# voletiv/mcvd-pytorch

Hardware: AMD Instinct MI355X
Metric: sampled frames/sec (whole node), SMMNIST 64x64 DDPM 100-step (higher is better)
Workload: dtype f32-equivalent: f32 storage and accumulation; 58 of 58 3x3 convs, 41 of 41 1x1 convs and the attention products (head dims 32..128) as SIX bf16 piece products of operands split EXACTLY into three bf16 pieces (all 24 bits, fp32 exponent range, less than one fp32 rounding per product; tests/test_gpu_p

## Files before the change

mcvd_pytorch_amd/csrc/kernels/conv_wino3.cpp:

```cpp
#include <stdlib.h>

#include "../common.h"
#include "conv_wino3_stage.h"

namespace mcvd {

#define W3_SLOT_OFF(word) (word)

template <int COT, int PRO, bool G8, int EXP = 0>
__global__ __launch_bounds__(512) __attribute__((amdgpu_num_vgpr(86))) void conv_wino3_kernel(ConvArgs a) {
    constexpr int NT = W3_NT, CK = W3_CK, T = W3_T, BCO = 32 * COT, PP = W3_PP, VW = W3_VW, PW = W3_PW;
    constexpr int PSZ = CK * 10 * PP;
    constexpr int PBUF = PSZ + 8;
    constexpr int NPL = G8 ? 1 : 3;
    constexpr int NPV = G8 ? 4 : 9;
    constexpr int NQ = 3 * COT;
    constexpr int NA = 2 * NQ;
    constexpr int VM_A = NQ + NPL;
    constexpr int PQ = 5;
    static_assert(NA <= 18 && NA > PQ, "named-register map of conv_wino3_stage.h: v172-v180 patch, v184-v255 eighteen weight quads");
    extern __shared__ __attribute__((aligned(16))) float smem[];
    unsigned* sV = reinterpret_cast<unsigned*>(smem);
    float* sP = smem + 2 * VW;
    float* sCo = sP + 2 * PBUF;

    {
        float top;
        asm volatile("" : "={v255}"(top));
    }
    asm volatile("" :: "s"(a.x0), "s"(a.x1), "s"(a.coef), "s"(a.wpb), "s"(a.B), "s"(a.H), "s"(a.W), "s"(a.Cin), "s"(a.CinP), "s"(a.C0),
                 "s"(a.C1), "s"(a.CoutP), "s"(a.ksplit), "s"(a.dbg), "s"(a.wdma));
    const unsigned long long t_start = a.dbg ? __builtin_amdgcn_s_memtime() : 0ull;
    const int tid = threadIdx.x, lane = tid & 63, wave = tid >> 6, l31 = lane & 31, half = lane >> 5;
    const int H = a.H, W = a.W, HW = H * W, Cin = a.Cin;
    const int nch_all = a.CinP / CK;
    const int ksp = a.ksplit >= 2 ? a.ksplit : 1, kh = ksp >= 2 ? (int)blockIdx.y : 0;
    const int c_begin = kh * (nch_all / ksp), c_end = c_begin + nch_all / ksp;
    const int PC = (nch_all / ksp) * CK;
    unsigned* sOff = reinterpret_cast<unsigned*>(sCo + (G8 ? 4 : 2) * PC);
    const int rx_n = G8 ? 1 : W >> 4, ry_n = G8 ? 1 : H >> 3;
    const int nreg = G8 ? (a.B + 1) >> 1 : a.B * rx_n * ry_n;
    const int nct = a.CoutP / BCO;
    const int xcd = blockIdx.x & 7, slot = blockIdx.x >> 3;
    const int reg_id = (slot / nct) * 8 + xcd;
    const int cotile = slot - (slot / nct) * nct;
    if (reg_id >= nreg) return;
    const int b = G8 ? 2 * reg_id : reg_id / (rx_n * ry_n);
    const int rr = G8 ? 0 : reg_id - b * (rx_n * ry_n);
    const int oy0 = (rr / rx_n) * 8, ox0 = (rr % rx_n) * 16;
    const int co0 = cotile * BCO;
    const int rg = __builtin_amdgcn_readfirstlane(wave >> 2);

    constexpr int NE = G8 ? 2 : 4;
    const bool wide = !G8 && PC > 2 * NT;
    const float* co_src[4];
#pragma unroll
    for (int k = 0; k < NE; ++k) {
        co_src[k] = a.coef + ((long)b * Cin + min(CK * c_begin + tid + k * NT, Cin - 1)) * 2;
        if (G8) co_src[2 + k] = a.coef + ((long)min(b + 1, a.B - 1) * Cin + min(CK * c_begin + tid + k * NT, Cin - 1)) * 2;
    }
    if (PRO) {
        asm volatile("global_load_dwordx2 v[172:173], %0, off\n\tglobal_load_dwordx2 v[174:175], %1, off"
                     :: "v"(co_src[0]), "v"(co_src[1]) : "memory");
        if (G8 || wide)
            asm volatile("global_load_dwordx2 v[176:177], %0, off\n\tglobal_load_dwordx2 v[178:179], %1, off"
                         :: "v"(co_src[2]), "v"(co_src[3]) : "memory");
    }

    const int s_tile = tid & 31, s_cp = (tid & 255) >> 5;
    const int s_ty = G8 ? (s_tile >> 2) & 3 : s_tile >> 3, s_tx = G8 ? (s_tile & 3) + 5 * (s_tile >> 4) : s_tile & 7;
    const int p_rd = ((s_cp * 10 + 2 * s_ty + rg) * PP + 2 * s_tx) * 2;
    const int v_wr = ((8 * rg * 2 + (s_cp & 1)) * 4 + (s_cp >> 1)) * T + s_tile;

    unsigned p_pk[NPL];
#pragma unroll
    for (int sl = 0; sl < NPL; ++sl) {
        p_pk[sl] = (unsigned)PSZ | ((unsigned)CK << 12);
        unsigned off = 0;
        if (G8) {
            const int e = tid, ci = e >> 5, img = (e >> 4) & 1, r = (e >> 1) & 7, c = (e & 1) * 4;
            const bool valid = b + img < a.B;
            const int cp = (ci >> 2) * 2 + (ci & 1), ce = (ci >> 1) & 1;
            p_pk[sl] = (unsigned)(((cp * 10 + r + 1) * PP + img * 10 + c + 1) * 2 + ce) | ((unsigned)(ci + (valid ? 0 : CK)) << 12) |
                       ((unsigned)(valid ? img : 0) << 20);
            off = (unsigned)(ci * HW + r * 8 + c) * 4u;
        } else if (sl < 2) {
            const int e = sl * NT + tid;
            if (e < CK * 40) {
                const int ci = e / 40, rem = e - ci * 40, r = rem >> 2, c = (rem & 3) * 4;
                const int y = oy0 - 1 + r;
                const bool inside = y >= 0 && y < H;
                const int cp = (ci >> 2) * 2 + (ci & 1), ce = (ci >> 1) & 1;
                p_pk[sl] = (unsigned)(((cp * 10 + r) * PP + c + 1) * 2 + ce) | ((unsigned)(ci + (inside ? 0 : CK)) << 12);
                off = (unsigned)(ci * HW + min(max(y, 0), H - 1) * W + ox0 + c) * 4u;
            }
        } else if (tid < CK * 20) {
            const int e = tid, ci = e / 20, rem = e - ci * 20, r = rem >> 1, c = (rem & 1) * 17;
            const int y = oy0 - 1 + r, x = ox0 - 1 + c;
            const bool inside = y >= 0 && y < H && x >= 0 && x < W;
            const int cp = (ci >> 2) * 2 + (ci & 1), ce = (ci >> 1) & 1;
            p_pk[sl] = (unsigned)(((cp * 10 + r) * PP + c) * 2 + ce) | ((unsigned)(ci + (inside ? 0 : CK)) << 12);
            off = (unsigned)(ci * HW + min(max(y, 0), H - 1) * W + min(max(x, 0), W - 1)) * 4u;
        }
        sOff[sl * NT + tid] = off;
    }

    const int wave_u = __builtin_amdgcn_readfirstlane(wave);
    const unsigned* wr_base = reinterpret_cast<const unsigned*>(a.wpb) + ((long)cotile * (a.CinP / CK) * 16 + 2 * wave_u) * (NQ * 256);
    const unsigned wr_voff = (unsigned)lane * 16u;

#define W3_WCHUNK(ch) (wr_base + (long)(ch) * (16 * NQ * 256))
#define W3_READ_OFF(OFS) { _Pragma("unroll") for (int sl = 0; sl < NPL; ++sl) OFS[sl] = sOff[sl * NT + tid]; }
#define W3_READ_C(ch, cfv)                                                                                      \
    {                                                                                                           \
        _Pragma("unroll") for (int sl = 0; sl < NPL; ++sl) {                                                    \
            cfv[sl] = f32x2{1.0f, 0.0f};                                                                        \
            if (PRO >= 1) {                                                                                     \
                 \
                const int cch = min(((ch) - c_begin) * CK + (int)((p_pk[sl] >> 12) & (CK - 1)), PC - 1) + (G8 ? (int)((p_pk[sl] >> 20) & 1u) * PC : 0); \
                cfv[sl] = *reinterpret_cast<const f32x2*>(sCo + cch * 2);                                       \
            }                                                                                                   \
        }                                                                                                       \
    }
                                                                                         \
#define W3_VALU_PHASE(ch, RG)                                                                                   \
    {                                                                                                           \
        {                                                                                                       \
            f32x2 cfv[NPL];                                                                                     \
            unsigned ofs[NPL];                                                                                  \
            W3_TS(7)                                                                                            \
            if (!(EXP & 2)) W3_READ_C((ch) + 2, cfv)                                                            \
            if (!(EXP & 4)) W3_READ_OFF(ofs)                                                                    \
            if (!(EXP & 4)) W3_WAIT(NA)                                                                         \
            W3_TS(0)                                                                                            \
            float pv[NPV];                                                                                      \
// ... 22 lines not shown
    const bool rec = a.dbg != nullptr && wave == (a.wdma & 7);
    const bool sub = (a.wdma & 64) != 0;
    unsigned long long sp[5] = {0, 0, 0, 0, 0};
    unsigned long long tk0 = 0, tprev = 0, dt[2] = {0, 0}, rt0 = 0;
    if (rec) {
        rt0 = __builtin_amdgcn_s_memrealtime();
        tk0 = tprev = t_start;
    }
#define W3_STAMP(i)                                                                                             \
    if (rec) {                                                                                                  \
        const unsigned long long now = __builtin_amdgcn_s_memtime();                                            \
        dt[i] += now - tprev;                                                                                   \
        tprev = now;                                                                                            \
    }
#ifdef MCVD_DIAG
    const bool tsub = rec && (a.wdma & 128) != 0;
    unsigned long long ts[8] = {0, 0, 0, 0, 0, 0, 0, 0}, tsp = 0;
#define W3_TS(i)                                                                                                \
    if (tsub) {                                                                                                 \
        const unsigned long long now = __builtin_amdgcn_s_memtime();                                            \
        ts[i] += now - tsp;                                                                                     \
        tsp = now;                                                                                              \
    }
#else
#define W3_TS(i)
#endif

    int vtok = 0;
    {
        const float nodep = 0.0f;
        unsigned ofs[NPL];
        W3_READ_OFF(ofs)
        if (rec) sp[3] = __builtin_amdgcn_s_memtime() - tk0;
        W3_LOAD_PR(b, c_begin, nodep, ofs, "v[184:187]", "v[188:191]", "v192")
        W3_LOAD_PR(b, c_begin + 1, nodep, ofs, "v[194:197]", "v[198:201]", "v202")
        if (G8)
            for (int i = tid; i < 2 * PBUF; i += NT) sP[i] = 0.0f;
        if (rec) sp[0] = __builtin_amdgcn_s_memtime() - tk0;
        W3_WAIT(0)
        if (rec) sp[1] = __builtin_amdgcn_s_memtime() - tk0;
        float cdep = 0.0f;
        if (PRO) {
            f32x2 cpre[4] = {{1.0f, 0.0f}, {1.0f, 0.0f}, {1.0f, 0.0f}, {1.0f, 0.0f}};
            asm volatile("v_mov_b32 %0, v172\n\tv_mov_b32 %1, v173\n\tv_mov_b32 %2, v174\n\tv_mov_b32 %3, v175"
                         : "=v"(cpre[0].x), "=v"(cpre[0].y), "=v"(cpre[1].x), "=v"(cpre[1].y) : "s"(vtok));
            if (G8 || wide)
                asm volatile("v_mov_b32 %0, v176\n\tv_mov_b32 %1, v177\n\tv_mov_b32 %2, v178\n\tv_mov_b32 %3, v179"
                             : "=v"(cpre[2].x), "=v"(cpre[2].y), "=v"(cpre[3].x), "=v"(cpre[3].y) : "s"(vtok));
#pragma unroll
            for (int k = 0; k < NE; ++k)
                if (tid + k * NT < PC) {
                    *reinterpret_cast<f32x2*>(sCo + (tid + k * NT) * 2) = cpre[k];
                    if constexpr (G8) *reinterpret_cast<f32x2*>(sCo + (PC + tid + k * NT) * 2) = cpre[2 + k];
                }
            cdep = cpre[0].x + cpre[1].x + cpre[2].x + cpre[3].x;
        }
        W3_LOAD_P(b, c_begin + 2, cdep, ofs)
        if (PRO || G8) __syncthreads();
        if (rec) sp[4] = __builtin_amdgcn_s_memtime() - tk0;
        {
            constexpr int QR = (NA - PQ + 2 * NPV - 1) / (2 * NPV);
#define W3_HOOK0(e, v) W3_LOAD_A_RANGE(W3_WCHUNK(c_begin), PQ + (e) * QR, (PQ + ((e) + 1) * QR < NA ? PQ + ((e) + 1) * QR : NA), v)
#define W3_HOOK1(e, v) W3_LOAD_A_RANGE(W3_WCHUNK(c_begin), (PQ + (NPV + (e)) * QR < NA ? PQ + (NPV + (e)) * QR : NA), (PQ + (NPV + (e) + 1) * QR < NA ? PQ + (NPV + (e) + 1) * QR : NA), v)
            float pv0[NPV], pv1[NPV];
            f32x2 cf0[NPL], cf1[NPL];
            W3_READ_C(c_begin, cf0)
            W3_READ_C(c_begin + 1, cf1)
            W3_WRITE_PR(c_begin & 1, Cin - c_begin * CK, 0u, pv0, cf0, "v184", "v185", "v186", "v187", "v188", "v189", "v190", "v191", "v192", W3_HOOK0)
            W3_WRITE_PR((c_begin + 1) & 1, Cin - (c_begin + 1) * CK, 0u, pv1, cf1, "v194", "v195", "v196", "v197", "v198", "v199", "v200", "v201", "v202", W3_HOOK1)
#undef W3_HOOK0
#undef W3_HOOK1
            const float dep = pv0[0] + pv1[0];
            W3_LOAD_A_RANGE(W3_WCHUNK(c_begin), 0, PQ, dep)
        }
    }
    __syncthreads();
    if (rec) sp[2] = __builtin_amdgcn_s_memtime() - tk0;
    {
        f32x2 rw[3][4];
        W3_READ_R(c_begin & 1, rw)
        W3_WRITE_V(c_begin & 1, rg, rw)
    }
    __syncthreads();
    W3_STAMP(0)

    W3_WAIT(0)
    const int ph = rg;
    if (ph == 0) {
        for (int c = c_begin; c + 1 < c_end; ++c) {
            W3_VALU_PHASE(c, rg)
            W3_MFMA_PHASE(c & 1, true, W3_WCHUNK(c + 1))
            asm volatile("s_waitcnt lgkmcnt(0)\n\ts_barrier" ::: "memory");
            W3_TS(6)
        }
    } else {
        for (int c = c_begin; c + 1 < c_end; ++c) {
            W3_MFMA_PHASE(c & 1, true, W3_WCHUNK(c + 1))
            W3_VALU_PHASE(c, rg)
            asm volatile("s_waitcnt lgkmcnt(0)\n\ts_barrier" ::: "memory");
            W3_TS(6)
        }
    }
    W3_WAIT(0)
    {
// ... 196 lines not shown
```

mcvd_pytorch_amd/csrc/kernels/conv_wino3_stage.h:

```cpp
#ifdef W3_STAGE_UNDEF
#undef W3_QUADS
#undef W3_LD1
#undef W3_LD1D
#undef W3_MF1
#undef W3_LOAD_A
#undef W3_LOAD_A_PIECE
#undef W3_LOAD_A_RANGE
#undef W3_WAIT
#undef W3_LOAD_PR
#undef W3_LOAD_P
#undef W3_NOHOOK
#undef W3_WRITE_PR
#undef W3_WRITE_P
#undef W3_READ_R
#undef W3_WRITE_V
#undef W3_LOAD_B
#undef W3_PRODUCT
#undef W3_MFMA_PHASE
#undef W3_STAGE_UNDEF
#else

#include "wino_common.h"

namespace mcvd {

constexpr int W3_CK = 16;
constexpr int W3_T = 32;
constexpr int W3_NT = 512;
#ifndef MCVD_W3_PP
#define MCVD_W3_PP 24
#endif
constexpr int W3_PP = MCVD_W3_PP;
constexpr int W3_PW = 16 * 2 * 4 * W3_T;
constexpr int W3_VW = 3 * W3_PW;

}

#define W3_QUADS(X, q, A1, A2) X(0, "v[184:187]", q, A1, A2) X(1, "v[188:191]", q, A1, A2) X(2, "v[192:195]", q, A1, A2) X(3, "v[196:199]", q, A1, A2) X(4, "v[200:203]", q, A1, A2) X(5, "v[204:207]", q, A1, A2) X(6, "v[208:211]", q, A1, A2) X(7, "v[212:215]", q, A1, A2) X(8, "v[216:219]", q, A1, A2) X(9, "v[220:223]", q, A1, A2) X(10, "v[224:227]", q, A1, A2) X(11, "v[228:231]", q, A1, A2) X(12, "v[232:235]", q, A1, A2) X(13, "v[236:239]", q, A1, A2) X(14, "v[240:243]", q, A1, A2) X(15, "v[244:247]", q, A1, A2) X(16, "v[248:251]", q, A1, A2) X(17, "v[252:255]", q, A1, A2)
#define W3_LD1(K, R, q, P, UNUSED) if ((q) == K) asm volatile("global_load_dwordx4 " R ", %0, %1" :: "v"(wr_voff), "s"(P) : "memory");
#define W3_MF1(K, R, q, ACC, BV) if ((q) == K) asm volatile("v_mfma_f32_32x32x16_bf16 %0, " R ", %1, %0" : "+v"(ACC) : "v"(BV));
#define W3_LOAD_A(WPTR, i)                                                                                      \
    {                                                                                                           \
        const unsigned* ua = (WPTR) + (i) * (NQ * 256);                                                         \
        _Pragma("unroll") for (int qq = 0; qq < NQ; ++qq) { W3_QUADS(W3_LD1, (i) * NQ + qq, ua + qq * 256, 0) } \
    }
#define W3_LOAD_A_PIECE(WPTR, i, pc)                                                                            \
    {                                                                                                           \
        const unsigned* ua = (WPTR) + (i) * (NQ * 256);                                                         \
        _Pragma("unroll") for (int ct = 0; ct < COT; ++ct) { W3_QUADS(W3_LD1, (i) * NQ + ct * 3 + (pc), ua + (ct * 3 + (pc)) * 256, 0) } \
    }
#define W3_LD1D(K, R, q, P, DEP) if ((q) == K) asm volatile("global_load_dwordx4 " R ", %0, %1" :: "v"(wr_voff), "s"(P), "v"(DEP) : "memory");
#define W3_LOAD_A_RANGE(WPTR, Q0, Q1, DEP)                                                                      \
    {                                                                                                           \
        const unsigned* ua = (WPTR);                                                                            \
        _Pragma("unroll") for (int qq = (Q0); qq < (Q1); ++qq) { W3_QUADS(W3_LD1D, qq, ua + qq * 256, DEP) }    \
    }
#define W3_WAIT(N) asm volatile("s_waitcnt vmcnt(%1)\n\ts_mov_b32 %0, 0" : "=s"(vtok) : "n"(N) : "memory");
#define W3_LOAD_PR(bb, ch, DEP, OFS, RA, RB, RH)                                                                \
    {                                                                                                           \
        const int cb = min((ch) * CK, Cin - 1);                                                                 \
        const unsigned lim4 = (unsigned)((Cin - cb) * HW - 4) * 4u, lim1 = (unsigned)((Cin - cb) * HW - 1) * 4u; \
        const bool second = cb >= a.C0;                                                                         \
        const float* srcb = second ? a.x1 + ((long)(bb) * a.C1 + (cb - a.C0)) * HW : a.x0 + ((long)(bb) * a.C0 + cb) * HW; \
         \
        if constexpr (G8) {                                                                                     \
            const unsigned istride = (unsigned)((second ? a.C1 : a.C0) * HW) * 4u;       \
            const unsigned o0 = min(W3_SLOT_OFF(OFS[0]), lim4) + ((p_pk[0] >> 20) & 1u) * istride;              \
            asm volatile("global_load_dwordx4 " RA ", %0, %1" :: "v"(o0), "s"(srcb), "v"(DEP) : "memory");     \
        } else {                                                                                                \
            const unsigned o0 = min(W3_SLOT_OFF(OFS[0]), lim4), o1 = min(W3_SLOT_OFF(OFS[NPL > 1 ? 1 : 0]), lim4),  \
                           o2 = min(W3_SLOT_OFF(OFS[NPL > 2 ? 2 : 0]), lim1);                                   \
            asm volatile("global_load_dwordx4 " RA ", %0, %3\n\tglobal_load_dwordx4 " RB ", %1, %3\n\tglobal_load_dword " RH ", %2, %3" \
                         :: "v"(o0), "v"(o1), "v"(o2), "s"(srcb), "v"(DEP) : "memory");                           \
        }                                                                                                       \
    }
#define W3_LOAD_P(bb, ch, DEP, OFS) W3_LOAD_PR(bb, ch, DEP, OFS, "v[172:175]", "v[176:179]", "v180")
#define W3_NOHOOK(e, v)
#define W3_WRITE_P(par, NV, FL, PV, cfv) W3_WRITE_PR(par, NV, FL, PV, cfv, "v172", "v173", "v174", "v175", "v176", "v177", "v178", "v179", "v180", W3_NOHOOK)
#define W3_WRITE_PR(par, NV, FL, PV, cfv, A0, A1, A2, A3, B0, B1, B2, B3, H0, HOOK)                             \
    {                                                                                                           \
        float* sPw = sP + ((par) ? PBUF : 0);                                                                   \
        const int nvalid = (NV);                                                                                \
         \
        if constexpr (G8) {                                                                                     \
            asm("v_fma_f32 %0, " A0 ", %4, %5\n\tv_fma_f32 %1, " A1 ", %4, %5\n\tv_fma_f32 %2, " A2 ", %4, %5\n\tv_fma_f32 %3, " A3 ", %4, %5" \
                : "=&v"(PV[0]), "=&v"(PV[1]), "=&v"(PV[2]), "=&v"(PV[3]) : "v"(cfv[0].x), "v"(cfv[0].y), "s"(vtok)); \
        } else {                                                                                                \
            asm("v_fma_f32 %0, " A0 ", %9, %10\n\tv_fma_f32 %1, " A1 ", %9, %10\n\tv_fma_f32 %2, " A2 ", %9, %10\n\tv_fma_f32 %3, " A3 ", %9, %10\n\t" \
                "v_fma_f32 %4, " B0 ", %11, %12\n\tv_fma_f32 %5, " B1 ", %11, %12\n\tv_fma_f32 %6, " B2 ", %11, %12\n\tv_fma_f32 %7, " B3 ", %11, %12\n\t" \
                "v_fma_f32 %8, " H0 ", %13, %14"                                                                  \
                : "=&v"(PV[0]), "=&v"(PV[1]), "=&v"(PV[2]), "=&v"(PV[3]), "=&v"(PV[4]), "=&v"(PV[5]), "=&v"(PV[6]), "=&v"(PV[7]), "=&v"(PV[NPV > 8 ? 8 : 0]) \
                : "v"(cfv[0].x), "v"(cfv[0].y), "v"(cfv[NPL > 1 ? 1 : 0].x), "v"(cfv[NPL > 1 ? 1 : 0].y), "v"(cfv[NPL > 2 ? 2 : 0].x), \
                  "v"(cfv[NPL > 2 ? 2 : 0].y), "s"(vtok));                                                        \
        }                                                                                                       \
        _Pragma("unroll") for (int e = 0; e < NPV; ++e) {                                                       \
            const int sl = e >> 2;                               \
            float v = PV[e];                                                                                    \
            if (PRO >= 2) v = wino_silu(v);                                                                     \
            const bool keep = (((FL) >> sl) & 1u) == 0u && (int)((p_pk[sl] >> 12) & 0xff) < min(nvalid, CK);    \
            sPw[(p_pk[sl] & 0xfff) + 2 * (e & 3)] = keep ? v : 0.0f;                                            \
            HOOK(e, v)                                                                                          \
        }                                                                                                       \
    }
#define W3_READ_R(par, RW)                                                                                      \
    {                                                                                                           \
        const f32x2* sPr = reinterpret_cast<const f32x2*>(sP + ((par) ? PBUF : 0) + p_rd);                      \
        _Pragma("unroll") for (int j = 0; j < 4; ++j) { RW[0][j] = sPr[j]; RW[1][j] = sPr[PP + j]; RW[2][j] = sPr[2 * PP + j]; } \
    }
#define W3_WRITE_V(par, RG, RW)                                                                                 \
    {                                                                                                           \
        unsigned* vdst = sV + ((par) ? VW : 0) + v_wr;                                                          \
        f32x2 mx[4], my[4];                                                                                     \
        _Pragma("unroll") for (int j = 0; j < 4; ++j) {                                                         \
            const f32x2 r0 = RW[0][j], r1 = RW[1][j], r2 = RW[2][j];                                            \
            if ((RG) == 0) { mx[j] = r0 - r2; my[j] = r1 + r2; }                                                \
            else { mx[j] = r1 - r0; my[j] = r0 - r2; }                                                          \
        }                                                                                                       \
        _Pragma("unroll") for (int row = 0; row < 2; ++row) {                                                   \
            const f32x2 m0 = row ? my[0] : mx[0], m1 = row ? my[1] : mx[1], m2 = row ? my[2] : mx[2], m3 = row ? my[3] : mx[3]; \
            const f32x2 v0 = m0 - m2, v1 = m1 + m2, v2 = m2 - m1, v3 = m1 - m3;                                 \
            _Pragma("unroll") for (int q = 0; q < 4; ++q) {                                                     \
                unsigned w1, w2, w3;                                                                            \
                wino_split3(q == 0 ? v0 : q == 1 ? v1 : q == 2 ? v2 : v3, w1, w2, w3);                          \
                vdst[(row * 4 + q) * 256] = w1;                                                                 \
                vdst[(row * 4 + q) * 256 + PW] = w2;                                                            \
                vdst[(row * 4 + q) * 256 + 2 * PW] = w3;                                                        \
            }                                                                                                   \
        }                                                                                                       \
    }
#define W3_LOAD_B(i, BQ)                                                                                        \
    {                                                                                                           \
        const unsigned* q = sVc + (((2 * wave + (i)) * 2 + half) * 4) * T + l31;                                \
        _Pragma("unroll") for (int jp = 0; jp < 4; ++jp) {                                                      \
// ... 32 lines not shown
```

mcvd_pytorch_amd/csrc/kernels/conv_wino3p.cpp:

```cpp
#include <stdlib.h>

#include "../common.h"
#include "conv_wino3_stage.h"

namespace mcvd {

constexpr int WP_NPL = 3;
constexpr int WP_MINCH = 4;

#define W3_SLOT_OFF(word) ((word) & ~3u)
#define W3_TS(i)

template <int COT, int PRO>
__global__ __launch_bounds__(512) __attribute__((amdgpu_num_vgpr(86))) void conv_wino3p_kernel(ConvArgs a) {
    constexpr int NT = W3_NT, CK = W3_CK, T = W3_T, BCO = 32 * COT, PP = W3_PP, VW = W3_VW, PW = W3_PW;
    constexpr int PSZ = CK * 10 * PP;
    constexpr int PBUF = 4096;
    static_assert(PBUF >= PSZ + 8 && PBUF >= 4 * 32 * W3_T, "patch buffer: patch + dump space, and 4 positions x 32 couts x 32 tiles of the epilogue");
    constexpr int NPL = WP_NPL, NPV = 9;
    constexpr bool G8 = false;
    constexpr int EXP = 0;
    constexpr int NQ = 3 * COT;
    constexpr int NA = 2 * NQ;
    constexpr int VM_A = NQ + NPL;
    constexpr int PQ = 5;
    constexpr long WSTR = 16L * NQ * 256;
    static_assert(NA <= 18 && NA > PQ, "named-register map of conv_wino3_stage.h: v172-v180 patch, v184-v255 eighteen weight quads");
    extern __shared__ __attribute__((aligned(16))) float smem[];
    unsigned* sV = reinterpret_cast<unsigned*>(smem);
    float* sP = smem + 2 * VW;
    float* sCo = sP + 2 * PBUF;
    unsigned* sOff = reinterpret_cast<unsigned*>(sCo + 2 * a.Cin);
    {
        float top;
        asm volatile("" : "={v255}"(top));
    }
    asm volatile("" :: "s"(a.x0), "s"(a.x1), "s"(a.coef), "s"(a.wpb), "s"(a.B), "s"(a.H), "s"(a.W), "s"(a.Cin), "s"(a.CinP), "s"(a.C0),
                 "s"(a.C1), "s"(a.CoutP), "s"(a.ksplit), "s"(a.dbg), "s"(a.wdma));
    const unsigned long long t_start = a.dbg ? __builtin_amdgcn_s_memtime() : 0ull;
    const int tid = threadIdx.x, lane = tid & 63, wave = tid >> 6, l31 = lane & 31, half = lane >> 5;
    const int H = a.H, W = a.W, HW = H * W, Cin = a.Cin;
    const int rx_n = W >> 4, rpi = rx_n * (H >> 3);
    const int nct = a.CoutP / BCO;
    const int ksp = a.ksplit >= 2 ? a.ksplit : 1;
    const int nch = (a.CinP / CK) / ksp;
    const int ips = rpi * nct * ksp;
    const int n_items = a.B * ips;
    const int it0 = (int)((long)blockIdx.x * n_items / gridDim.x), it1 = (int)((long)(blockIdx.x + 1) * n_items / gridDim.x);
    if (it0 >= it1) return;
    const int rg = __builtin_amdgcn_readfirstlane(wave >> 2);
    const int wave_u = __builtin_amdgcn_readfirstlane(wave);
#ifdef MCVD_DIAG
    if ((a.wdma >> 8) != 0 && (blockIdx.x & 1)) {
        const unsigned long long until = __builtin_amdgcn_s_memtime() + ((unsigned long long)(a.wdma >> 8) << 8);
        while (__builtin_amdgcn_s_memtime() < until) __builtin_amdgcn_s_sleep(8);
    }
#endif

    const int s_tile = tid & 31, s_cp = (tid & 255) >> 5;
    const int s_ty = s_tile >> 3, s_tx = s_tile & 7;
    const int p_rd = ((s_cp * 10 + 2 * s_ty + rg) * PP + 2 * s_tx) * 2;
    const int v_wr = ((8 * rg * 2 + (s_cp & 1)) * 4 + (s_cp >> 1)) * T + s_tile;

    unsigned p_pk[NPL];
#pragma unroll
    for (int sl = 0; sl < NPL; ++sl) {
        p_pk[sl] = (unsigned)PSZ | ((unsigned)CK << 12);
        if (sl < 2) {
            const int e = sl * NT + tid;
            if (e < CK * 40) {
                const int ci = e / 40, rem = e - ci * 40, r = rem >> 2, c = (rem & 3) * 4;
                const int cp = (ci >> 2) * 2 + (ci & 1), ce = (ci >> 1) & 1;
                p_pk[sl] = (unsigned)(((cp * 10 + r) * PP + c + 1) * 2 + ce) | ((unsigned)ci << 12);
            }
        } else if (tid < CK * 20) {
            const int e = tid, ci = e / 20, rem = e - ci * 20, r = rem >> 1, c = (rem & 1) * 17;
            const int cp = (ci >> 2) * 2 + (ci & 1), ce = (ci >> 1) & 1;
            p_pk[sl] = (unsigned)(((cp * 10 + r) * PP + c) * 2 + ce) | ((unsigned)ci << 12);
        }
    }
#define WP_SLOT_TABLE(tab, oy0, ox0, OUT)                                                                       \
    {                                                                                                           \
        int tid_s;        \
        asm volatile("v_mov_b32 %0, %1" : "=v"(tid_s) : "v"(tid));                                              \
        _Pragma("unroll") for (int sl = 0; sl < NPL; ++sl) {                                                    \
            unsigned off = 1u;                                                                                  \
            if (sl < 2) {                                                                                       \
                const int e = sl * NT + tid_s;                                                                  \
                if (e < CK * 40) {                                                                              \
                    const int ci = e / 40, rem = e - ci * 40, r = rem >> 2, c = (rem & 3) * 4;                  \
                    const int y = (oy0) - 1 + r;                                                                \
                    const bool inside = y >= 0 && y < H;                                                        \
                    off = (unsigned)(ci * HW + min(max(y, 0), H - 1) * W + (ox0) + c) * 4u + (inside ? 0u : 1u); \
                }                                                                                               \
            } else if (tid_s < CK * 20) {                                                                       \
                const int e = tid_s, ci = e / 20, rem = e - ci * 20, r = rem >> 1, c = (rem & 1) * 17;          \
                const int y = (oy0) - 1 + r, x = (ox0) - 1 + c;                                                 \
                const bool inside = y >= 0 && y < H && x >= 0 && x < W;                                         \
                off = (unsigned)(ci * HW + min(max(y, 0), H - 1) * W + min(max(x, 0), W - 1)) * 4u + (inside ? 0u : 1u); \
            }                                                                                                   \
            sOff[((tab) * NPL + sl) * NT + tid] = off;                                                          \
            OUT[sl] = off;                                                                                      \
        }                                                                                                       \
    }

    const unsigned wr_voff = (unsigned)lane * 16u;

#define WP_READ_C(ch, cfv)                                                                                      \
    {                                                                                                           \
        _Pragma("unroll") for (int sl = 0; sl < NPL; ++sl) {                                                    \
            cfv[sl] = f32x2{1.0f, 0.0f};                                                                        \
            if (PRO >= 1) {                                                                                     \
                const int cch = min((ch) * CK + (int)((p_pk[sl] >> 12) & (CK - 1)), Cin - 1);                   \
                cfv[sl] = *reinterpret_cast<const f32x2*>(sCo + cch * 2);                                       \
            }                                                                                                   \
        }                                                                                                       \
    }
#define WP_VALU_PHASE(par, CH2, CH3, TAB3, RG)                                                                  \
    {                                                                                                           \
        {                                                                                                       \
            f32x2 cfv[NPL];                                                                                     \
            unsigned ofs[NPL];                                                                                  \
            WP_READ_C(CH2, cfv)                                                                                 \
            _Pragma("unroll") for (int sl = 0; sl < NPL; ++sl) ofs[sl] = sOff[((TAB3) * NPL + sl) * NT + tid];  \
            W3_WAIT(NA)                                                                                         \
            float pv[NPV];                                                                                      \
            _Pragma("unroll") for (int e = 0; e < NPV; ++e) pv[e] = 0.0f;                                       \
            W3_WRITE_P(par, min(Cin - (CH2) * CK, CK), pfl, pv, cfv)                                            \
            pfl = (ofs[0] & 1u) | ((ofs[1] & 1u) << 1) | ((ofs[2] & 1u) << 2);                                  \
            W3_LOAD_P(b, CH3, pv[0], ofs)                                                                       \
        }                                                                                                       \
        {                                                                                                       \
            f32x2 rw[3][4];                                                                                     \
// ... 14 lines not shown
    unsigned long long tprev = t_start, dt[3] = {0, 0, 0}, rt0 = 0;
    if (rec) rt0 = __builtin_amdgcn_s_memrealtime();
#define WP_STAMP(i)                                                                                             \
    if (rec) {                                                                                                  \
        const unsigned long long now = __builtin_amdgcn_s_memtime();                                            \
        dt[i] += now - tprev;                                                                                   \
        tprev = now;                                                                                            \
    }

    const unsigned* const wpb_u = reinterpret_cast<const unsigned*>(a.wpb);
    const bool fin = ksp == 1;
    int vtok = 0;
    unsigned pfl = 0;
    int chunks_done = 0;

    int it = it0;
    while (it < it1) {
        const int b = it / ips;
        const int run_end = min(it1, (b + 1) * ips);
        {
            const int q0 = it - b * ips, kh = q0 % ksp, q1 = q0 / ksp, cotile = q1 % nct, rr = q1 / nct;
            const int oy0 = (rr / rx_n) * 8, ox0 = (rr % rx_n) * 16, cbeg = kh * nch;
            const unsigned* w0 = wpb_u + (((long)cotile * (nch * ksp) + cbeg) * 16 + 2 * wave_u) * (NQ * 256);
            const float* co_src[2];
#pragma unroll
            for (int k = 0; k < 2; ++k) co_src[k] = a.coef + ((long)b * Cin + min(tid + k * NT, Cin - 1)) * 2;
            if (PRO)
                asm volatile("global_load_dwordx2 v[172:173], %0, off\n\tglobal_load_dwordx2 v[174:175], %1, off"
                             :: "v"(co_src[0]), "v"(co_src[1]) : "memory");
            const float nodep = 0.0f;
            unsigned ofs[NPL];
            WP_SLOT_TABLE(it & 1, oy0, ox0, ofs)
            const unsigned fl0 = (ofs[0] & 1u) | ((ofs[1] & 1u) << 1) | ((ofs[2] & 1u) << 2);
            W3_LOAD_PR(b, cbeg, nodep, ofs, "v[184:187]", "v[188:191]", "v192")
            W3_LOAD_PR(b, cbeg + 1, nodep, ofs, "v[194:197]", "v[198:201]", "v202")
            W3_WAIT(0)
            float cdep = 0.0f;
            if (PRO) {
                f32x2 cpre[2];
                asm volatile("v_mov_b32 %0, v172\n\tv_mov_b32 %1, v173\n\tv_mov_b32 %2, v174\n\tv_mov_b32 %3, v175"
                             : "=v"(cpre[0].x), "=v"(cpre[0].y), "=v"(cpre[1].x), "=v"(cpre[1].y) : "s"(vtok));
#pragma unroll
                for (int k = 0; k < 2; ++k)
                    if (tid + k * NT < Cin) *reinterpret_cast<f32x2*>(sCo + (tid + k * NT) * 2) = cpre[k];
                cdep = cpre[0].x + cpre[1].x;
            }
            W3_LOAD_P(b, cbeg + 2, cdep, ofs)
            pfl = fl0;
            if (PRO) asm volatile("s_waitcnt lgkmcnt(0)\n\ts_barrier" ::: "memory");
            {
                constexpr int QR = (NA - PQ + 2 * NPV - 1) / (2 * NPV);
#define WP_HOOK0(e, v) W3_LOAD_A_RANGE(w0, PQ + (e) * QR, (PQ + ((e) + 1) * QR < NA ? PQ + ((e) + 1) * QR : NA), v)
#define WP_HOOK1(e, v) W3_LOAD_A_RANGE(w0, (PQ + (NPV + (e)) * QR < NA ? PQ + (NPV + (e)) * QR : NA), (PQ + (NPV + (e) + 1) * QR < NA ? PQ + (NPV + (e) + 1) * QR : NA), v)
                float pv0[NPV], pv1[NPV];
                f32x2 cf0[NPL], cf1[NPL];
                WP_READ_C(cbeg, cf0)
                WP_READ_C(cbeg + 1, cf1)
                W3_WRITE_PR(0, min(Cin - cbeg * CK, CK), fl0, pv0, cf0, "v184", "v185", "v186", "v187", "v188", "v189", "v190", "v191", "v192", WP_HOOK0)
                W3_WRITE_PR(1, min(Cin - (cbeg + 1) * CK, CK), fl0, pv1, cf1, "v194", "v195", "v196", "v197", "v198", "v199", "v200", "v201", "v202", WP_HOOK1)
#undef WP_HOOK0
#undef WP_HOOK1
                const float dep = pv0[0] + pv1[0];
                W3_LOAD_A_RANGE(w0, 0, PQ, dep)
            }
            asm volatile("s_waitcnt lgkmcnt(0)\n\ts_barrier" ::: "memory");
            {
                f32x2 rw[3][4];
                W3_READ_R(0, rw)
                W3_WRITE_V(0, rg, rw)
            }
            asm volatile("s_waitcnt lgkmcnt(0)\n\ts_barrier" ::: "memory");
            W3_WAIT(0)
        }
        WP_STAMP(0)
        int par = 0;
        for (; it < run_end; ++it) {
            const int q0 = it - b * ips, kh = q0 % ksp, q1 = q0 / ksp, cotile = q1 % nct, rr = q1 / nct;
            const int nx = it + 1 < run_end ? it + 1 : it;
            const int n0 = nx - b * ips, nkh = n0 % ksp, n1 = n0 / ksp, ncotile = n1 % nct, nrr = n1 / nct;
            const int cbeg = kh * nch, ncbeg = nkh * nch;
            const unsigned* wb_cur = wpb_u + (((long)cotile * (nch * ksp) + cbeg) * 16 + 2 * wave_u) * (NQ * 256);
            const unsigned* wb_nx = wpb_u + (((long)ncotile * (nch * ksp) + ncbeg) * 16 + 2 * wave_u) * (NQ * 256);
            const int tab_cur = it & 1, tab_nx = nx & 1;
            {
                unsigned dummy[NPL];
                WP_SLOT_TABLE(tab_nx, (nrr / rx_n) * 8, (nrr % rx_n) * 16, dummy)
                (void)dummy;
            }
#define WP_CHUNK_SCALARS                                                                                        \
            const int l2 = c + 2, l3 = c + 3;                                                                   \
            const int ch2 = l2 < nch ? cbeg + l2 : ncbeg + l2 - nch;                                            \
            const int ch3 = l3 < nch ? cbeg + l3 : ncbeg + l3 - nch;                                            \
            const int tab3 = l3 < nch ? tab_cur : tab_nx;                                                       \
            const unsigned* wnx = c + 1 < nch ? wb_cur + (long)(c + 1) * WSTR : wb_nx;
// ... 159 lines not shown
```

Measured before the change: 262.9.

## Remap Winograd patch slots to one quad plus two singles per thread

Result: no change. 264.8, median of 6 (+0.7%).

```diff
diff --git a/mcvd_pytorch_amd/csrc/kernels/conv_wino3.cpp b/mcvd_pytorch_amd/csrc/kernels/conv_wino3.cpp
--- a/mcvd_pytorch_amd/csrc/kernels/conv_wino3.cpp
+++ b/mcvd_pytorch_amd/csrc/kernels/conv_wino3.cpp
@@ -12,13 +12,13 @@
     constexpr int NT = W3_NT, CK = W3_CK, T = W3_T, BCO = 32 * COT, PP = W3_PP, VW = W3_VW, PW = W3_PW;
     constexpr int PSZ = CK * 10 * PP;
     constexpr int PBUF = PSZ + 8;
-    constexpr int NPL = G8 ? 1 : 3;
-    constexpr int NPV = G8 ? 4 : 9;
+    constexpr int NPL = G8 ? 1 : wino_slots::NSLOT;
+    constexpr int NPV = G8 ? 4 : wino_slots::NVAL;
     constexpr int NQ = 3 * COT;
     constexpr int NA = 2 * NQ;
     constexpr int VM_A = NQ + NPL;
-    constexpr int PQ = 5;
-    static_assert(NA <= 18 && NA > PQ, "named-register map of conv_wino3_stage.h: v172-v180 patch, v184-v255 eighteen weight quads");
+    constexpr int PQ = G8 ? 5 : 3;
+    static_assert(NA <= 18 && NA > PQ, "named-register map of conv_wino3_stage.h: v172-v176, v180 patch, v184-v255 eighteen weight quads");
     extern __shared__ __attribute__((aligned(16))) float smem[];
     unsigned* sV = reinterpret_cast<unsigned*>(smem);
     float* sP = smem + 2 * VW;
@@ -84,23 +84,11 @@
             p_pk[sl] = (unsigned)(((cp * 10 + r + 1) * PP + img * 10 + c + 1) * 2 + ce) | ((unsigned)(ci + (valid ? 0 : CK)) << 12) |
                        ((unsigned)(valid ? img : 0) << 20);
             off = (unsigned)(ci * HW + r * 8 + c) * 4u;
-        } else if (sl < 2) {
-            const int e = sl * NT + tid;
-            if (e < CK * 40) {
-                const int ci = e / 40, rem = e - ci * 40, r = rem >> 2, c = (rem & 3) * 4;
-                const int y = oy0 - 1 + r;
-                const bool inside = y >= 0 && y < H;
-                const int cp = (ci >> 2) * 2 + (ci & 1), ce = (ci >> 1) & 1;
-                p_pk[sl] = (unsigned)(((cp * 10 + r) * PP + c + 1) * 2 + ce) | ((unsigned)(ci + (inside ? 0 : CK)) << 12);
-                off = (unsigned)(ci * HW + min(max(y, 0), H - 1) * W + ox0 + c) * 4u;
-            }
-        } else if (tid < CK * 20) {
-            const int e = tid, ci = e / 20, rem = e - ci * 20, r = rem >> 1, c = (rem & 1) * 17;
-            const int y = oy0 - 1 + r, x = ox0 - 1 + c;
-            const bool inside = y >= 0 && y < H && x >= 0 && x < W;
-            const int cp = (ci >> 2) * 2 + (ci & 1), ce = (ci >> 1) & 1;
-            p_pk[sl] = (unsigned)(((cp * 10 + r) * PP + c) * 2 + ce) | ((unsigned)(ci + (inside ? 0 : CK)) << 12);
-            off = (unsigned)(ci * HW + min(max(y, 0), H - 1) * W + min(max(x, 0), W - 1)) * 4u;
+        } else {
+            const wino_slots::Slot ws = wino_slots::slot(sl, tid);
+            const wino_slots::SlotSource src = wino_slots::slot_source(ws, oy0, ox0, H, W);
+            p_pk[sl] = (unsigned)wino_slots::slot_lds_index(PP, ws) | ((unsigned)(ws.ch + (src.inside ? 0 : CK)) << 12);
+            off = src.off;
         }
         sOff[sl * NT + tid] = off;
     }
@@ -189,8 +177,13 @@
         unsigned ofs[NPL];
         W3_READ_OFF(ofs)
         if (rec) sp[3] = __builtin_amdgcn_s_memtime() - tk0;
-        W3_LOAD_PR(b, c_begin, nodep, ofs, "v[184:187]", "v[188:191]", "v192")
-        W3_LOAD_PR(b, c_begin + 1, nodep, ofs, "v[194:197]", "v[198:201]", "v202")
+        if constexpr (G8) {
+            W3_LOAD_PR(b, c_begin, nodep, ofs, "v[184:187]", "", "")
+            W3_LOAD_PR(b, c_begin + 1, nodep, ofs, "v[194:197]", "", "")
+        } else {
+            W3_LOAD_PR(b, c_begin, nodep, ofs, "v[184:187]", "v188", "v189")
+            W3_LOAD_PR(b, c_begin + 1, nodep, ofs, "v[190:193]", "v194", "v195")
+        }
         if (G8)
             for (int i = tid; i < 2 * PBUF; i += NT) sP[i] = 0.0f;
         if (rec) sp[0] = __builtin_amdgcn_s_memtime() - tk0;
@@ -217,16 +210,24 @@
         if (rec) sp[4] = __builtin_amdgcn_s_memtime() - tk0;
         {
             constexpr int QR = (NA - PQ + 2 * NPV - 1) / (2 * NPV);
-#define W3_HOOK0(e, v) W3_LOAD_A_RANGE(W3_WCHUNK(c_begin), PQ + (e) * QR, (PQ + ((e) + 1) * QR < NA ? PQ + ((e) + 1) * QR : NA), v)
-#define W3_HOOK1(e, v) W3_LOAD_A_RANGE(W3_WCHUNK(c_begin), (PQ + (NPV + (e)) * QR < NA ? PQ + (NPV + (e)) * QR : NA), (PQ + (NPV + (e) + 1) * QR < NA ? PQ + (NPV + (e) + 1) * QR : NA), v)
+#define W3_HQ(g) (G8 ? (PQ + (g) * QR < NA ? PQ + (g) * QR : NA) : PQ + (g) * (NA - PQ) / (2 * NPV))
+#define W3_HOOK0(e, v) W3_LOAD_A_RANGE(W3_WCHUNK(c_begin), W3_HQ(e), W3_HQ((e) + 1), v)
+#define W3_HOOK1(e, v) W3_LOAD_A_RANGE(W3_WCHUNK(c_begin), W3_HQ(NPV + (e)), W3_HQ(NPV + (e) + 1), v)
+            static_assert(W3_HQ(0) == PQ && W3_HQ(2 * NPV) == NA, "every quad from PQ up is requested behind a value, in order");
             float pv0[NPV], pv1[NPV];
             f32x2 cf0[NPL], cf1[NPL];
             W3_READ_C(c_begin, cf0)
             W3_READ_C(c_begin + 1, cf1)
-            W3_WRITE_PR(c_begin & 1, Cin - c_begin * CK, 0u, pv0, cf0, "v184", "v185", "v186", "v187", "v188", "v189", "v190", "v191", "v192", W3_HOOK0)
-            W3_WRITE_PR((c_begin + 1) & 1, Cin - (c_begin + 1) * CK, 0u, pv1, cf1, "v194", "v195", "v196", "v197", "v198", "v199", "v200", "v201", "v202", W3_HOOK1)
+            if constexpr (G8) {
+                W3_WRITE_PR(c_begin & 1, Cin - c_begin * CK, 0u, pv0, cf0, "v184", "v185", "v186", "v187", "", "", W3_HOOK0)
+                W3_WRITE_PR((c_begin + 1) & 1, Cin - (c_begin + 1) * CK, 0u, pv1, cf1, "v194", "v195", "v196", "v197", "", "", W3_HOOK1)
+            } else {
+                W3_WRITE_PR(c_begin & 1, Cin - c_begin * CK, 0u, pv0, cf0, "v184", "v185", "v186", "v187", "v188", "v189", W3_HOOK0)
+                W3_WRITE_PR((c_begin + 1) & 1, Cin - (c_begin + 1) * CK, 0u, pv1, cf1, "v190", "v191", "v192", "v193", "v194", "v195", W3_HOOK1)
+            }
 #undef W3_HOOK0
 #undef W3_HOOK1
+#undef W3_HQ
             const float dep = pv0[0] + pv1[0];
             W3_LOAD_A_RANGE(W3_WCHUNK(c_begin), 0, PQ, dep)
         }
diff --git a/mcvd_pytorch_amd/csrc/kernels/conv_wino3_stage.h b/mcvd_pytorch_amd/csrc/kernels/conv_wino3_stage.h
--- a/mcvd_pytorch_amd/csrc/kernels/conv_wino3_stage.h
+++ b/mcvd_pytorch_amd/csrc/kernels/conv_wino3_stage.h
@@ -21,6 +21,7 @@
 #else
 
 #include "wino_common.h"
+#include "wino_slots.h"
 
 namespace mcvd {
 
@@ -33,6 +34,7 @@
 constexpr int W3_PP = MCVD_W3_PP;
 constexpr int W3_PW = 16 * 2 * 4 * W3_T;
 constexpr int W3_VW = 3 * W3_PW;
+static_assert(W3_CK == wino_slots::CK && W3_NT == wino_slots::NT && wino_slots::lds_exact(W3_PP), "the slot map's chunk, thread count and patch pitch are the kernels'");
 
 }
 
@@ -68,16 +70,16 @@
             const unsigned o0 = min(W3_SLOT_OFF(OFS[0]), lim4) + ((p_pk[0] >> 20) & 1u) * istride;              \
             asm volatile("global_load_dwordx4 " RA ", %0, %1" :: "v"(o0), "s"(srcb), "v"(DEP) : "memory");     \
         } else {                                                                                                \
-            const unsigned o0 = min(W3_SLOT_OFF(OFS[0]), lim4), o1 = min(W3_SLOT_OFF(OFS[NPL > 1 ? 1 : 0]), lim4),  \
+            const unsigned o0 = min(W3_SLOT_OFF(OFS[0]), lim4), o1 = min(W3_SLOT_OFF(OFS[NPL > 1 ? 1 : 0]), lim1),  \
                            o2 = min(W3_SLOT_OFF(OFS[NPL > 2 ? 2 : 0]), lim1);                                   \
-            asm volatile("global_load_dwordx4 " RA ", %0, %3\n\tglobal_load_dwordx4 " RB ", %1, %3\n\tglobal_load_dword " RH ", %2, %3" \
+            asm volatile("global_load_dwordx4 " RA ", %0, %3\n\tglobal_load_dword " RB ", %1, %3\n\tglobal_load_dword " RH ", %2, %3" \
                          :: "v"(o0), "v"(o1), "v"(o2), "s"(srcb), "v"(DEP) : "memory");                           \
         }                                                                                                       \
     }
-#define W3_LOAD_P(bb, ch, DEP, OFS) W3_LOAD_PR(bb, ch, DEP, OFS, "v[172:175]", "v[176:179]", "v180")
+#define W3_LOAD_P(bb, ch, DEP, OFS) W3_LOAD_PR(bb, ch, DEP, OFS, "v[172:175]", "v176", "v180")
 #define W3_NOHOOK(e, v)
-#define W3_WRITE_P(par, NV, FL, PV, cfv) W3_WRITE_PR(par, NV, FL, PV, cfv, "v172", "v173", "v174", "v175", "v176", "v177", "v178", "v179", "v180", W3_NOHOOK)
-#define W3_WRITE_PR(par, NV, FL, PV, cfv, A0, A1, A2, A3, B0, B1, B2, B3, H0, HOOK)                             \
+#define W3_WRITE_P(par, NV, FL, PV, cfv) W3_WRITE_PR(par, NV, FL, PV, cfv, "v172", "v173", "v174", "v175", "v176", "v180", W3_NOHOOK)
+#define W3_WRITE_PR(par, NV, FL, PV, cfv, A0, A1, A2, A3, S1, S2, HOOK)                                         \
     {                                                                                                           \
         float* sPw = sP + ((par) ? PBUF : 0);                                                                   \
         const int nvalid = (NV);                                                                                \
@@ -86,19 +88,18 @@
             asm("v_fma_f32 %0, " A0 ", %4, %5\n\tv_fma_f32 %1, " A1 ", %4, %5\n\tv_fma_f32 %2, " A2 ", %4, %5\n\tv_fma_f32 %3, " A3 ", %4, %5" \
                 : "=&v"(PV[0]), "=&v"(PV[1]), "=&v"(PV[2]), "=&v"(PV[3]) : "v"(cfv[0].x), "v"(cfv[0].y), "s"(vtok)); \
         } else {                                                                                                \
-            asm("v_fma_f32 %0, " A0 ", %9, %10\n\tv_fma_f32 %1, " A1 ", %9, %10\n\tv_fma_f32 %2, " A2 ", %9, %10\n\tv_fma_f32 %3, " A3 ", %9, %10\n\t" \
-                "v_fma_f32 %4, " B0 ", %11, %12\n\tv_fma_f32 %5, " B1 ", %11, %12\n\tv_fma_f32 %6, " B2 ", %11, %12\n\tv_fma_f32 %7, " B3 ", %11, %12\n\t" \
-                "v_fma_f32 %8, " H0 ", %13, %14"                                                                  \
-                : "=&v"(PV[0]), "=&v"(PV[1]), "=&v"(PV[2]), "=&v"(PV[3]), "=&v"(PV[4]), "=&v"(PV[5]), "=&v"(PV[6]), "=&v"(PV[7]), "=&v"(PV[NPV > 8 ? 8 : 0]) \
+            asm("v_fma_f32 %0, " A0 ", %6, %7\n\tv_fma_f32 %1, " A1 ", %6, %7\n\tv_fma_f32 %2, " A2 ", %6, %7\n\tv_fma_f32 %3, " A3 ", %6, %7\n\t" \
+                "v_fma_f32 %4, " S1 ", %8, %9\n\tv_fma_f32 %5, " S2 ", %10, %11"                                 \
+                : "=&v"(PV[0]), "=&v"(PV[1]), "=&v"(PV[2]), "=&v"(PV[3]), "=&v"(PV[NPV > 4 ? 4 : 0]), "=&v"(PV[NPV > 5 ? 5 : 0]) \
                 : "v"(cfv[0].x), "v"(cfv[0].y), "v"(cfv[NPL > 1 ? 1 : 0].x), "v"(cfv[NPL > 1 ? 1 : 0].y), "v"(cfv[NPL > 2 ? 2 : 0].x), \
                   "v"(cfv[NPL > 2 ? 2 : 0].y), "s"(vtok));                                                        \
         }                                                                                                       \
         _Pragma("unroll") for (int e = 0; e < NPV; ++e) {                                                       \
-            const int sl = e >> 2;                               \
+            const int sl = wino_slots::value_slot(e);              \
             float v = PV[e];                                                                                    \
             if (PRO >= 2) v = wino_silu(v);                                                                     \
             const bool keep = (((FL) >> sl) & 1u) == 0u && (int)((p_pk[sl] >> 12) & 0xff) < min(nvalid, CK);    \
-            sPw[(p_pk[sl] & 0xfff) + 2 * (e & 3)] = keep ? v : 0.0f;                                            \
+            sPw[(p_pk[sl] & 0xfff) + 2 * wino_slots::value_elem(e)] = keep ? v : 0.0f;                          \
             HOOK(e, v)                                                                                          \
         }                                                                                                       \
     }
diff --git a/mcvd_pytorch_amd/csrc/kernels/conv_wino3p.cpp b/mcvd_pytorch_amd/csrc/kernels/conv_wino3p.cpp
--- a/mcvd_pytorch_amd/csrc/kernels/conv_wino3p.cpp
+++ b/mcvd_pytorch_amd/csrc/kernels/conv_wino3p.cpp
@@ -5,7 +5,7 @@
 
 namespace mcvd {
 
-constexpr int WP_NPL = 3;
+constexpr int WP_NPL = wino_slots::NSLOT;
 constexpr int WP_MINCH = 4;
 
 #define W3_SLOT_OFF(word) ((word) & ~3u)
@@ -17,15 +17,15 @@
     constexpr int PSZ = CK * 10 * PP;
     constexpr int PBUF = 4096;
     static_assert(PBUF >= PSZ + 8 && PBUF >= 4 * 32 * W3_T, "patch buffer: patch + dump space, and 4 positions x 32 couts x 32 tiles of the epilogue");
-    constexpr int NPL = WP_NPL, NPV = 9;
+    constexpr int NPL = WP_NPL, NPV = wino_slots::NVAL;
     constexpr bool G8 = false;
     constexpr int EXP = 0;
     constexpr int NQ = 3 * COT;
     constexpr int NA = 2 * NQ;
     constexpr int VM_A = NQ + NPL;
-    constexpr int PQ = 5;
+    constexpr int PQ = 3;
     constexpr long WSTR = 16L * NQ * 256;
-    static_assert(NA <= 18 && NA > PQ, "named-register map of conv_wino3_stage.h: v172-v180 patch, v184-v255 eighteen weight quads");
+    static_assert(NA <= 18 && NA > PQ, "named-register map of conv_wino3_stage.h: v172-v176, v180 patch, v184-v255 eighteen weight quads");
     extern __shared__ __attribute__((aligned(16))) float smem[];
     unsigned* sV = reinterpret_cast<unsigned*>(smem);
     float* sP = smem + 2 * VW;
@@ -65,40 +65,16 @@
     unsigned p_pk[NPL];
 #pragma unroll
     for (int sl = 0; sl < NPL; ++sl) {
-        p_pk[sl] = (unsigned)PSZ | ((unsigned)CK << 12);
-        if (sl < 2) {
-            const int e = sl * NT + tid;
-            if (e < CK * 40) {
-                const int ci = e / 40, rem = e - ci * 40, r = rem >> 2, c = (rem & 3) * 4;
-                const int cp = (ci >> 2) * 2 + (ci & 1), ce = (ci >> 1) & 1;
-                p_pk[sl] = (unsigned)(((cp * 10 + r) * PP + c + 1) * 2 + ce) | ((unsigned)ci << 12);
-            }
-        } else if (tid < CK * 20) {
-            const int e = tid, ci = e / 20, rem = e - ci * 20, r = rem >> 1, c = (rem & 1) * 17;
-            const int cp = (ci >> 2) * 2 + (ci & 1), ce = (ci >> 1) & 1;
-            p_pk[sl] = (unsigned)(((cp * 10 + r) * PP + c) * 2 + ce) | ((unsigned)ci << 12);
-        }
+        const wino_slots::Slot ws = wino_slots::slot(sl, tid);
+        p_pk[sl] = (unsigned)wino_slots::slot_lds_index(PP, ws) | ((unsigned)ws.ch << 12);
     }
 #define WP_SLOT_TABLE(tab, oy0, ox0, OUT)                                                                       \
     {                                                                                                           \
         int tid_s;        \
         asm volatile("v_mov_b32 %0, %1" : "=v"(tid_s) : "v"(tid));                                              \
         _Pragma("unroll") for (int sl = 0; sl < NPL; ++sl) {                                                    \
-            unsigned off = 1u;                                                                                  \
-            if (sl < 2) {                                                                                       \
-                const int e = sl * NT + tid_s;                                                                  \
-                if (e < CK * 40) {                                                                              \
-                    const int ci = e / 40, rem = e - ci * 40, r = rem >> 2, c = (rem & 3) * 4;                  \
-                    const int y = (oy0) - 1 + r;                                                                \
-                    const bool inside = y >= 0 && y < H;                                                        \
-                    off = (unsigned)(ci * HW + min(max(y, 0), H - 1) * W + (ox0) + c) * 4u + (inside ? 0u : 1u); \
-                }                                                                                               \
-            } else if (tid_s < CK * 20) {                                                                       \
-                const int e = tid_s, ci = e / 20, rem = e - ci * 20, r = rem >> 1, c = (rem & 1) * 17;          \
-                const int y = (oy0) - 1 + r, x = (ox0) - 1 + c;                                                 \
-                const bool inside = y >= 0 && y < H && x >= 0 && x < W;                                         \
-                off = (unsigned)(ci * HW + min(max(y, 0), H - 1) * W + min(max(x, 0), W - 1)) * 4u + (inside ? 0u : 1u); \
-            }                                                                                                   \
+            const wino_slots::SlotSource src = wino_slots::slot_source(wino_slots::slot(sl, tid_s), oy0, ox0, H, W); \
+            const unsigned off = src.off + (src.inside ? 0u : 1u);         \
             sOff[((tab) * NPL + sl) * NT + tid] = off;                                                          \
             OUT[sl] = off;                                                                                      \
         }                                                                                                       \
@@ -179,8 +155,8 @@
             unsigned ofs[NPL];
             WP_SLOT_TABLE(it & 1, oy0, ox0, ofs)
             const unsigned fl0 = (ofs[0] & 1u) | ((ofs[1] & 1u) << 1) | ((ofs[2] & 1u) << 2);
-            W3_LOAD_PR(b, cbeg, nodep, ofs, "v[184:187]", "v[188:191]", "v192")
-            W3_LOAD_PR(b, cbeg + 1, nodep, ofs, "v[194:197]", "v[198:201]", "v202")
+            W3_LOAD_PR(b, cbeg, nodep, ofs, "v[184:187]", "v188", "v189")
+            W3_LOAD_PR(b, cbeg + 1, nodep, ofs, "v[190:193]", "v194", "v195")
             W3_WAIT(0)
             float cdep = 0.0f;
             if (PRO) {
@@ -196,17 +172,19 @@
             pfl = fl0;
             if (PRO) asm volatile("s_waitcnt lgkmcnt(0)\n\ts_barrier" ::: "memory");
             {
-                constexpr int QR = (NA - PQ + 2 * NPV - 1) / (2 * NPV);
-#define WP_HOOK0(e, v) W3_LOAD_A_RANGE(w0, PQ + (e) * QR, (PQ + ((e) + 1) * QR < NA ? PQ + ((e) + 1) * QR : NA), v)
-#define WP_HOOK1(e, v) W3_LOAD_A_RANGE(w0, (PQ + (NPV + (e)) * QR < NA ? PQ + (NPV + (e)) * QR : NA), (PQ + (NPV + (e) + 1) * QR < NA ? PQ + (NPV + (e) + 1) * QR : NA), v)
+#define WP_HQ(g) (PQ + (g) * (NA - PQ) / (2 * NPV))
+#define WP_HOOK0(e, v) W3_LOAD_A_RANGE(w0, WP_HQ(e), WP_HQ((e) + 1), v)
+#define WP_HOOK1(e, v) W3_LOAD_A_RANGE(w0, WP_HQ(NPV + (e)), WP_HQ(NPV + (e) + 1), v)
+                static_assert(WP_HQ(0) == PQ && WP_HQ(2 * NPV) == NA, "every quad from PQ up is requested behind a value, in order");
                 float pv0[NPV], pv1[NPV];
                 f32x2 cf0[NPL], cf1[NPL];
                 WP_READ_C(cbeg, cf0)
                 WP_READ_C(cbeg + 1, cf1)
-                W3_WRITE_PR(0, min(Cin - cbeg * CK, CK), fl0, pv0, cf0, "v184", "v185", "v186", "v187", "v188", "v189", "v190", "v191", "v192", WP_HOOK0)
-                W3_WRITE_PR(1, min(Cin - (cbeg + 1) * CK, CK), fl0, pv1, cf1, "v194", "v195", "v196", "v197", "v198", "v199", "v200", "v201", "v202", WP_HOOK1)
+                W3_WRITE_PR(0, min(Cin - cbeg * CK, CK), fl0, pv0, cf0, "v184", "v185", "v186", "v187", "v188", "v189", WP_HOOK0)
+                W3_WRITE_PR(1, min(Cin - (cbeg + 1) * CK, CK), fl0, pv1, cf1, "v190", "v191", "v192", "v193", "v194", "v195", WP_HOOK1)
 #undef WP_HOOK0
 #undef WP_HOOK1
+#undef WP_HQ
                 const float dep = pv0[0] + pv1[0];
                 W3_LOAD_A_RANGE(w0, 0, PQ, dep)
             }
diff --git a/mcvd_pytorch_amd/csrc/kernels/wino_slots.h b/mcvd_pytorch_amd/csrc/kernels/wino_slots.h
--- /dev/null
+++ b/mcvd_pytorch_amd/csrc/kernels/wino_slots.h
@@ -0,0 +1,114 @@
+#pragma once
+
+namespace mcvd {
+namespace wino_slots {
+
+constexpr int CK = 16;
+constexpr int ROWS = 10;
+constexpr int COLS = 18;
+constexpr int NT = 512;
+constexpr int NSLOT = 3;
+constexpr int NVAL = 6;
+constexpr int ITEMS = CK * ROWS * 4;
+constexpr int HALO = CK * ROWS * 2;
+
+struct Slot {
+    int ch, row, col;
+    int width;
+};
+
+constexpr Slot item_slot(int item, int px, int width) {
+    const int ci = item / 40, rem = item - ci * 40;
+    return Slot{ci, rem >> 2, 1 + (rem & 3) * 4 + px, width};
+}
+constexpr Slot slot(int sl, int tid) {
+    if (sl == 0) return item_slot(tid, 0, 4);
+    if (sl == 1) return item_slot(NT + (tid >> 2), tid & 3, 1);
+    if (tid < HALO) {
+        const int ci = tid / 20, rem = tid - ci * 20;
+        return Slot{ci, rem >> 1, (rem & 1) * (COLS - 1), 1};
+    }
+    return Slot{CK, 0, 0, 0};
+}
+
+constexpr int value_slot(int e) { return e < 4 ? 0 : e - 3; }
+constexpr int value_elem(int e) { return e < 4 ? e : 0; }
+
+constexpr int patch_floats(int pp) { return CK * ROWS * pp; }
+constexpr int lds_index(int pp, int ch, int row, int col) {
+    const int cp = (ch >> 2) * 2 + (ch & 1), ce = (ch >> 1) & 1;
+    return ((cp * ROWS + row) * pp + col) * 2 + ce;
+}
+constexpr int slot_lds_index(int pp, const Slot& s) { return s.width ? lds_index(pp, s.ch, s.row, s.col) : patch_floats(pp); }
+
+struct SlotSource {
+    unsigned off;
+    bool inside;
+};
+constexpr int clampi(int v, int lo, int hi) { return v < lo ? lo : v > hi ? hi : v; }
+constexpr SlotSource slot_source(const Slot& s, int oy0, int ox0, int H, int W) {
+    if (!s.width) return SlotSource{0u, false};
+    const int y = oy0 - 1 + s.row, x = ox0 - 1 + s.col;
+    const bool inside = y >= 0 && y < H && x >= 0 && x + s.width <= W;
+    return SlotSource{(unsigned)(s.ch * (H * W) + clampi(y, 0, H - 1) * W + clampi(x, 0, W - 1)) * 4u, inside};
+}
+
+constexpr bool cover_exact() {
+    int n[CK * ROWS * COLS] = {};
+    for (int sl = 0; sl < NSLOT; ++sl)
+        for (int t = 0; t < NT; ++t) {
+            const Slot s = slot(sl, t);
+            if (s.width != 0 && (s.ch < 0 || s.ch >= CK || s.row < 0 || s.row >= ROWS || s.col < 0 || s.col + s.width > COLS)) return false;
+            for (int k = 0; k < s.width; ++k) ++n[(s.ch * ROWS + s.row) * COLS + s.col + k];
+        }
+    for (int i = 0; i < CK * ROWS * COLS; ++i)
+        if (n[i] != 1) return false;
+    return true;
+}
+constexpr bool lds_exact(int pp) {
+    if (pp < COLS || patch_floats(pp) + 8 > 4096) return false;
+    bool seen[4096] = {};
+    for (int sl = 0; sl < NSLOT; ++sl)
+        for (int t = 0; t < NT; ++t) {
+            const Slot s = slot(sl, t);
+            if (!s.width && slot_lds_index(pp, s) != patch_floats(pp)) return false;
+            for (int k = 0; k < s.width; ++k) {
+                const int i = slot_lds_index(pp, s) + 2 * k;
+                if (i < 0 || i >= patch_floats(pp) || seen[i]) return false;
+                seen[i] = true;
+            }
+        }
+    return true;
+}
+constexpr bool six_values() {
+    for (int t = 0; t < NT; ++t) {
+        const int w0 = slot(0, t).width, w1 = slot(1, t).width, w2 = slot(2, t).width;
+        if (w0 != 4 || w1 > 1 || w2 > 1) return false;
+    }
+    int per_slot[NSLOT] = {};
+    for (int e = 0; e < NVAL; ++e) {
+        if (value_slot(e) < 0 || value_slot(e) >= NSLOT || value_elem(e) != per_slot[value_slot(e)]) return false;
+        ++per_slot[value_slot(e)];
+    }
+    return per_slot[0] == 4 && per_slot[1] == 1 && per_slot[2] == 1;
+}
+constexpr bool source_inside(int H, int W, int oy0, int ox0) {
+    for (int sl = 0; sl < NSLOT; ++sl)
+        for (int t = 0; t < NT; ++t) {
+            const Slot s = slot(sl, t);
+            const SlotSource src = slot_source(s, oy0, ox0, H, W);
+            if (src.off % 4u != 0u || (s.width == 4 && src.off % 16u != 0u)) return false;
+            if (s.width && src.off + 4u * (unsigned)s.width > (unsigned)(CK * H * W) * 4u) return false;
+        }
+    return true;
+}
+
+static_assert(ITEMS + 0 == 640 && HALO == 320 && 4 * NT + 4 * (ITEMS - NT) + HALO == CK * ROWS * COLS, "the census: 512 items, 512 singles of 128 items, 320 halo pixels");
+static_assert(cover_exact(), "the 512 x 3 slots cover each of the 16 x 10 x 18 patch elements exactly once");
+static_assert(lds_exact(24) && lds_exact(25) && lds_exact(18), "every parked value has its own LDS word inside the patch, at the committed pitch and the build variants'");
+static_assert(six_values(), "six values per thread: one four-pixel slot and two single-pixel slots");
+static_assert(source_inside(8, 16, 0, 0) && source_inside(64, 64, 0, 0) && source_inside(64, 64, 56, 48) && source_inside(32, 32, 8, 16) && source_inside(16, 32, 8, 0),
+              "clamped source offsets stay inside the chunk's planes: one-region plane, corners and interior");
+
+}
+}
```
